# hasnainfarid/Mujoco_Gymnasium_Environments

Hardware: AMD Instinct MI355X
Metric: env steps/sec (whole node), humanoid_soccer 4096 envs/GPU at 1/2/4/8 MI355X (higher is better)
Workload: dtype f64

## Files before the change

mujoco_gymnasium_environments_amd/csrc/mgx_api.hip:

```cpp
#include <hip/hip_runtime.h>

#include <cmath>
#include <cstdio>
#include <cstring>
#include <map>
#include <mutex>
#include <string>
#include <vector>

#include "mgx_task_host.h"

using namespace mgx;

MGX_PROF_SETTER(mgx_prof_set_buffer)

namespace {
thread_local std::string g_err;
}

namespace mgx {
int host_fail(int code, const std::string& msg) {
  g_err = msg;
  return code;
}
// ... 237 lines not shown
    L.hess = u0;
    L.con_pos = endA;
    L.con_frame = align_up(L.con_pos + 3 * max_ncon, al);
    endA = std::max(align_up(L.con_frame + 9 * max_ncon, al), align_up(u0 + (efcg ? nv * (nv + 1) / 2 : nv * nv), al));
  }
  int endB = align_up(u0 + L.chunk_rows * L.Bstride, al);
  L.reals = endA > endB ? endA : endB;
  int q = 0;
  auto takei = [&](int n) { int r = q; q = align_up(q + (n > 0 ? n : 1), 4); return r; };
  L.con_geom = takei(2 * max_ncon);
  L.carry_ints = q;
  L.con_pair = takei(max_ncon);
  L.act_list = takei(max_active);
  L.efc_type = takei(max_nefc); L.efc_id = takei(max_nefc);
  L.con_efcadr = takei(1);
  if (d->solver == 2 && takei(4) != team_off(L)) abort();
  L.ints = q;
  L.bytes = L.reals * real_bytes + L.ints * 4;
  (void)vec_end;
  return L;
}

Layout make_staged_layout(const mgx_model_desc* d, int real_bytes, int max_ncon, int max_nefc, int max_active,
                          int gcon) {
  Layout L{};
  int p = 0;
  const int al = 16 / real_bytes;
  auto a = [&](int n) { return align_up(n > 0 ? n : 1, al); };
  auto take = [&](int n) { int r = p; p += a(n); return r; };
  const int nb = d->nbody, nv = d->nv, nj = d->njnt, ng = d->ngeom;
  L.max_ncon = max_ncon; L.max_nefc = max_nefc; L.max_active = max_active;
  L.staged = 1;
  L.late_geom = 1;
  L.cfs = 3;
  L.qpos = take(d->nq); L.qvel = take(nv); L.ctrl = take(d->nu);
  L.xpos = take(3 * nb); L.xquat = take(4 * nb); L.subtree_com = take(3 * nb);
  L.qLD = take(d->nM); L.con_dist = take(max_ncon);
  L.carry_lds = p;
  L.con_mu = take(max_ncon); L.xfrc = take(6 * nb); L.qMH = take(d->nM);
  L.carry_reals = p;
  p = L.carry_lds;
  const int nvw = nv > 64 ? 128 : 64;
  L.vec0 = take(nvw); L.vec1 = take(nvw); L.vec2 = take(nvw); L.vec3 = take(nvw);
  L.cdof = take(6 * nv);
  L.efc = take(1); L.efc_margin = take(1); L.efc_blk = take(1);
  L.cvel = take(6 * nb);
  const int R = p;
  L.xipos = R; L.cinert = L.xipos + a(3 * nb); L.crb = L.cinert + a(10 * nb);
  const int dead = L.crb + a(10 * nb);
  L.xmat = dead; L.ximat = L.xmat + a(9 * nb); L.xaxis = L.ximat + a(9 * nb); L.xanchor = L.xaxis + a(3 * nj);
  const int endA1 = L.xanchor + a(3 * nj);
  L.cdof_dot = dead; L.cfrc = L.cdof_dot + a(6 * nv); L.act_force = L.cfrc + a(6 * nb);
  L.xfrc_lds = L.act_force + a(d->nu);
  const int endA2 = L.xfrc_lds + a(6 * nb);
  const int ecap = std::min(max_nefc, align_up(2 * nj, 4));
  const int nlist = std::max(max_active, ecap);
  L.geom_xpos = R; L.geom_xmat = L.geom_xpos + a(3 * ng);
  L.con_frame = L.geom_xmat + a(9 * ng);
  L.gcon = gcon;
  L.con_pos = gcon ? 0 : L.con_frame + a(3 * max_ncon);
  L.act_union = L.con_frame + a(3 * max_ncon) + (gcon ? 0 : a(3 * max_ncon));
  const int endC = L.act_union + a((nlist * 4 + real_bytes - 1) / real_bytes);
  L.cacc = a(12 * nb) <= L.con_frame - R ? R : endC;
  const int endD = L.cacc + a(12 * nb);
  L.reals = std::max(std::max(endA1, endA2), std::max(endC, endD));
  L.rowc = 0; L.rk = 0; L.hess = 0;
  L.Bstride = nv | 1; L.Bmat = R; L.chunk_rows = 0; L.gB = 0; L.gB_stride = 0; L.tchunk = 0;
  int q = 0;
  auto takei = [&](int n) { int r = q; q = align_up(q + (n > 0 ? n : 1), 4); return r; };
  L.con_geom = takei(2 * max_ncon);
  L.carry_ints = q;
  L.con_pair = takei(max_ncon);
  L.act_list = 0; L.efc_id = 0;
  L.efc_type = takei(1);
  L.con_efcadr = takei(1);
  L.ints = q;
  L.bytes = L.reals * real_bytes + L.ints * 4;
  return L;
}

Layout finisher_layout(const Layout& S, int real_bytes) {
  Layout L = S;
  const int nvw = S.vec1 - S.vec0;
  L.vec0 = S.carry_reals; L.vec1 = L.vec0 + nvw; L.vec2 = L.vec1 + nvw; L.vec3 = L.vec2 + nvw;
  L.carry_lds = S.carry_reals;
  L.reals = L.vec3 + nvw;
  L.ints = S.carry_ints;
  L.bytes = L.reals * real_bytes + L.ints * 4;
  return L;
}

template <typename T>
struct Builder {
  std::vector<char> host;
  std::vector<std::pair<size_t, const void**>> fix;
  size_t add(const void* src, size_t bytes, const void** slot) {
    size_t off = (host.size() + 15) / 16 * 16;
    host.resize(off + (bytes ? bytes : 16));
    if (bytes) memcpy(host.data() + off, src, bytes);
    fix.push_back({off, slot});
    return off;
  }
  template <typename S>
  void ints(const S* src, size_t n, const int** slot) {
    std::vector<int> v(n ? n : 1, 0);
    for (size_t i = 0; i < n; i++) v[i] = (int)src[i];
    add(v.data(), v.size() * 4, (const void**)slot);
  }
// ... 24 lines not shown
    depth[b] = (int)path.size();
    for (int c = 0; c < depth[b]; c++) chain[b * MGX_MAX_DEPTH + c] = path[depth[b] - 1 - c];
  }
  std::vector<int> chainlen(nv), anc(nv * MGX_MAX_DEPTH, -1), ancadr(nv * MGX_MAX_DEPTH, 0);
  std::vector<uint64_t> ancmask(nv, 0), ancmask_hi(nv, 0);
  for (int k = 0; k < nv; k++) {
    int t = 0;
    for (int j = k; j >= 0; j = d->dof_parentid[j], t++) {
      if (t >= MGX_MAX_DEPTH) return host_fail(MGX_E_CAPACITY, "dof chain longer than MGX_MAX_DEPTH");
      anc[k * MGX_MAX_DEPTH + t] = j;
      ancadr[k * MGX_MAX_DEPTH + t] = d->dof_Madr[j];
      if (j != k) {
        if (j < 64) ancmask[k] |= 1ull << j;
        else ancmask_hi[k] |= 1ull << (j - 64);
      }
    }
    chainlen[k] = t;
  }
  B.ints(d->body_parentid, nb, &M.body_parentid); B.ints(d->body_rootid, nb, &M.body_rootid);
  B.ints(d->body_jntnum, nb, &M.body_jntnum); B.ints(d->body_jntadr, nb, &M.body_jntadr);
  B.ints(d->body_dofnum, nb, &M.body_dofnum); B.ints(d->body_dofadr, nb, &M.body_dofadr);
  B.ints(d->body_subtree_end, nb, &M.body_subtree_end); B.ints(chain.data(), chain.size(), &M.body_chain);
  B.ints(depth.data(), nb, &M.body_depth);
  B.add(d->body_dofmask, sizeof(uint32_t) * nb * d->nmaskword, (const void**)&M.body_dofmask);
  B.reals(d->body_pos, 3 * nb, &M.body_pos); B.reals(d->body_quat, 4 * nb, &M.body_quat);
  B.reals(d->body_ipos, 3 * nb, &M.body_ipos); B.reals(d->body_iquat, 4 * nb, &M.body_iquat);
  B.reals(d->body_mass, nb, &M.body_mass); B.reals(d->body_inertia, 3 * nb, &M.body_inertia);
  B.reals(d->body_invweight0, 2 * nb, &M.body_invweight0);
  B.ints(d->jnt_type, nj, &M.jnt_type); B.ints(d->jnt_bodyid, nj, &M.jnt_bodyid);
  B.ints(d->jnt_qposadr, nj, &M.jnt_qposadr); B.ints(d->jnt_dofadr, nj, &M.jnt_dofadr);
  B.ints(d->jnt_limited, nj, &M.jnt_limited);
  B.reals(d->jnt_pos, 3 * nj, &M.jnt_pos); B.reals(d->jnt_axis, 3 * nj, &M.jnt_axis);
  B.reals(d->jnt_range, 2 * nj, &M.jnt_range); B.reals(d->jnt_stiffness, nj, &M.jnt_stiffness);
  B.reals(d->jnt_margin, nj, &M.jnt_margin); B.reals(d->jnt_solref, 2 * nj, &M.jnt_solref);
  B.reals(d->jnt_solimp, 5 * nj, &M.jnt_solimp);
  B.ints(d->dof_bodyid, nv, &M.dof_bodyid); B.ints(d->dof_jntid, nv, &M.dof_jntid);
  B.ints(d->dof_parentid, nv, &M.dof_parentid); B.ints(d->dof_Madr, nv, &M.dof_Madr);
  B.ints(chainlen.data(), nv, &M.dof_chainlen); B.ints(anc.data(), anc.size(), &M.dof_anc);
  B.add(ancmask.data(), 8 * ancmask.size(), (const void**)&M.dof_ancmask);
  B.add(ancmask_hi.data(), 8 * ancmask_hi.size(), (const void**)&M.dof_ancmask_hi);
  B.ints(ancadr.data(), ancadr.size(), &M.dof_ancadr);
  B.reals(d->dof_armature, nv, &M.dof_armature); B.reals(d->dof_damping, nv, &M.dof_damping);
  B.reals(d->dof_invweight0, nv, &M.dof_invweight0);
  B.ints(d->geom_type, ng, &M.geom_type); B.ints(d->geom_bodyid, ng, &M.geom_bodyid);
  B.reals(d->geom_size, 3 * ng, &M.geom_size); B.reals(d->geom_pos, 3 * ng, &M.geom_pos);
  B.reals(d->geom_quat, 4 * ng, &M.geom_quat); B.reals(d->geom_rbound, ng, &M.geom_rbound);
// ... 241 lines not shown
  };
  h.pgs_lds_rows = get("MGX_PGS_LDS_ROWS", 0);
  h.rk_lds_rows = get("MGX_RK_LDS_ROWS", 0);
  h.pgs_single = get("MGX_PGS_SINGLE", 0);
  h.pgs_lds_b = get("MGX_PGS_LDS_B", MGX_PGS_LDS_B) != 0;
  h.pgs_arena = get("MGX_PGS_ARENA", 0);
  h.pgs_lds_pad = get("MGX_PGS_LDS_PAD", 0);
  h.pgs_wide_lds = get("MGX_PGS_WIDE_LDS", 1);
  h.pgs_spw = get("MGX_PGS_SPW", 0);
  h.pgs_prio_rows = get("MGX_PGS_PRIO_ROWS", 0);
  h.pgs_split_blocks = get("MGX_PGS_SPLIT_BLOCKS", -1);
  h.tight_bp = get("MGX_TIGHT_BROADPHASE", -1);
  h.pgs_wpc = get("MGX_PGS_WPC", 4);
  if (h.pgs_wpc < 4 || h.pgs_wpc > 16) h.pgs_wpc = 4;
  h.side_stream = get("MGX_SIDE_STREAM", 1) != 0;
  h.bank_stream = get("MGX_BANK_STREAM", -1);
  if (h.bank_stream < -1 || h.bank_stream > 2) h.bank_stream = 0;
  h.tail_finish = get("MGX_TAIL_FINISH", -1);
  if (h.tail_finish < -1 || h.tail_finish > 1) h.tail_finish = 0;
  h.tail_factor = get("MGX_TAIL_FACTOR", 1);
  if (h.tail_factor < 0 || h.tail_factor > 2) h.tail_factor = 1;
  h.gcon = get("MGX_GCON", 1);
  h.rows_lds = get("MGX_ROWS_LDS", 0);
  return h;
}

SideStream* mgx::side_stream(hipStream_t st) {
  static std::mutex mu;
  static std::map<std::pair<hipStream_t, int>, SideStream*> cache;
  int dev = 0;
  if (hipGetDevice(&dev) != hipSuccess) return nullptr;
  std::lock_guard<std::mutex> lock(mu);
  auto key = std::make_pair(st, dev);
  auto it = cache.find(key);
  if (it != cache.end()) return it->second;
  SideStream* x = new SideStream{};
  if (hipStreamCreateWithFlags(&x->s, hipStreamNonBlocking) != hipSuccess ||
      hipEventCreateWithFlags(&x->rows, hipEventDisableTiming) != hipSuccess ||
      hipEventCreateWithFlags(&x->big, hipEventDisableTiming) != hipSuccess) {
    delete x;
    x = nullptr;
  }
  cache[key] = x;
  return x;
}

// ... 217 lines not shown
  }
  if (const char* v = getenv("MGX_MAX_NCON")) {
    if (atoi(v) < max_ncon) { delete m; return host_fail(MGX_E_ARG, "MGX_MAX_NCON below the model's contact capacity"); }
    max_ncon = atoi(v);
  }
  if (max_nefc > 1024 || max_ncon > 512) { delete m; return host_fail(MGX_E_CAPACITY, "capacity above 1024 rows / 512 contacts"); }
  max_nefc = (max_nefc + 3) & ~3;
  if (max_nefc < 4 || max_ncon < 1) { delete m; return host_fail(MGX_E_ARG, "row / contact capacity too small"); }
  int rb = precision == MGX_F32 ? 4 : 8;
  int max_active = d->npair <= 256 ? 128 : (d->npair < 768 ? d->npair : 768);
  m->staged_ok = d->integrator == 0 && d->solver == 0 && max_nefc <= 64 * MGX_EFC_SLOTS && condim13 &&
                 d->nv <= 56;
  m->staged_rk_ok = d->integrator == 1 && d->solver == 0 && condim13 && d->nv > 48 && d->nv <= 64 &&
                    max_nefc <= 1024 && max_ncon <= 192;
  const bool mono_lds_rows = !(d->layout_flags & MGX_ROWS_IN_SCRATCH);
  const int mono_nefc = m->staged_ok && mono_lds_rows && max_nefc > 192 ? 192
                        : (m->staged_rk_ok && max_nefc > 512 ? 512 : max_nefc);
  const int mono_ncon = m->staged_ok && mono_lds_rows && max_ncon > 64 ? 64 : max_ncon;
  m->L = make_layout(d, rb, mono_ncon, mono_nefc, max_active);
  if (m->L.bytes > 160 * 1024 || (d->layout_flags & MGX_ROWS_IN_SCRATCH))
    m->L = make_layout(d, rb, mono_ncon, mono_nefc, max_active, true);
  const bool any_staged = m->staged_ok || m->staged_rk_ok;
  m->Ls = make_staged_layout(d, rb, max_ncon, any_staged ? max_nefc : 4, m->staged_ok ? 128 : max_active,
                             m->hooks.gcon);
  m->Lf = finisher_layout(m->Ls, rb);
  {
    const int tight = m->hooks.tight_bp >= 0 ? (m->hooks.tight_bp != 0) : (d->npair > MGX_TIGHT_BROADPHASE_PAIRS);
    m->L.tight_bp = m->Ls.tight_bp = m->Lf.tight_bp = tight;
  }
  int rc;
  if (precision == MGX_F32) {
    rc = build_model<float>(d, device, m, m->mf);
    m->mf.L = m->L; m->mfs = m->mf; m->mfs.L = m->Ls; m->mff = m->mf; m->mff.L = m->Lf;
  } else {
    rc = build_model<double>(d, device, m, m->md);
    m->md.L = m->L; m->mds = m->md; m->mds.L = m->Ls; m->mdf = m->md; m->mdf.L = m->Lf;
  }
  if (rc != MGX_OK) { delete m; return rc; }
  if (m->L.bytes > 160 * 1024) { delete m; return host_fail(MGX_E_CAPACITY, "per-env LDS exceeds 160 KiB"); }
  int r2 = step_kernels_configure(m);
  if (r2 != MGX_OK) { delete m; return r2; }
  r2 = forward_kernels_configure(m);
  if (r2 != MGX_OK) { delete m; return r2; }
  r2 = dyn_kernels_configure(m);
  if (r2 != MGX_OK) { delete m; return r2; }
  r2 = ik_kernels_configure(m);
  if (r2 != MGX_OK) { delete m; return r2; }
// ... 139 lines not shown
```

mujoco_gymnasium_environments_amd/csrc/mgx_common.h:

```cpp
#pragma once
#include <hip/hip_runtime.h>
#include <stdint.h>

#define MGX_WAVE 64
#define MGX_MAX_NV 64
#define MGX_MAX_NV_WIDE 128
#define MGX_MAX_NBODY 64
#define MGX_MAX_DEPTH 16
#define MGX_MAX_CONPAIR 8
#define MGX_TIGHT_BROADPHASE_PAIRS 200
#define MGX_EFC_SLOTS 6

namespace mgx {

enum { JFREE = 0, JBALL = 1, JSLIDE = 2, JHINGE = 3 };
enum { GPLANE = 0, GHFIELD = 1, GSPHERE = 2, GCAPSULE = 3, GELLIPSOID = 4, GCYLINDER = 5, GBOX = 6 };
enum { C_LIMIT_JOINT = 3, C_CONTACT_FRICTIONLESS = 5, C_CONTACT_PYRAMIDAL = 6 };

struct Layout {
  int qpos, qvel, ctrl, xfrc, xpos, xquat, xmat, xipos, ximat, subtree_com, cinert, crb, cvel, cfrc;
  int xaxis, xanchor, cdof, cdof_dot, qLD, qMH, vec0, vec1, vec2, vec3, geom_xpos, geom_xmat, act_force, cacc, rowc;
  int con_dist, con_pos, con_frame, con_mu;
  int efc, efc_margin, efc_blk;
  int Bmat, Bstride;
  int reals;
  int con_geom, con_pair, act_list, efc_type, efc_id, con_efcadr;
  int ints;
  int bytes;
  int max_ncon, max_nefc, max_active;
  int staged, carry_reals, carry_ints, chunk_rows;
  int rk;
  int gB, gB_stride;
  int tchunk;
  int hess;
  int act_union;
  int carry_lds;
  int late_geom, cfs;
  int tight_bp;
  int xfrc_lds;
  int gcon;
};
__host__ __device__ inline int mgx_align(int x, int a) { return (x + a - 1) / a * a; }
__host__ __device__ inline int gb_efc_off(const Layout& L, int real_bytes) {
  return mgx_align(L.max_nefc * L.Bstride, 16 / real_bytes);
}
__host__ __device__ inline int gb_efm_off(const Layout& L, int real_bytes) {
  return gb_efc_off(L, real_bytes) + mgx_align(8 * L.max_nefc, 16 / real_bytes);
}
__host__ __device__ inline int team_off(const Layout& L) { return L.con_efcadr + 4; }

template <typename T>
struct DevModel {
  int nq, nv, nu, nbody, njnt, ngeom, npair, nM, nmaskword;
  int solver, integrator, cone, iterations;
  int has_damping;
  T timestep, tolerance, impratio, meaninertia, gravity[3];
  const int *body_parentid, *body_rootid, *body_jntnum, *body_jntadr, *body_dofnum, *body_dofadr;
  const int *body_subtree_end, *body_chain, *body_depth;
  const uint32_t *body_dofmask;
  const T *body_pos, *body_quat, *body_ipos, *body_iquat, *body_mass, *body_inertia, *body_invweight0;
  const int *jnt_type, *jnt_bodyid, *jnt_qposadr, *jnt_dofadr, *jnt_limited;
  const T *jnt_pos, *jnt_axis, *jnt_range, *jnt_stiffness, *jnt_margin, *jnt_solref, *jnt_solimp;
  const int *dof_bodyid, *dof_jntid, *dof_parentid, *dof_Madr, *dof_chainlen, *dof_anc;
  const uint64_t *dof_ancmask;
  const uint64_t *dof_ancmask_hi;
  const int *dof_ancadr;
  const T *dof_armature, *dof_damping, *dof_invweight0;
  const int *geom_type, *geom_bodyid;
  const T *geom_size, *geom_pos, *geom_quat, *geom_rbound;
  const int *pair_geom, *pair_condim;
  const int* pair_bpi;
  const T* pair_bpr;
  const T* geom_obb;
  const T *pair_friction, *pair_margin, *pair_gap, *pair_solref, *pair_solimp;
  const int *actuator_trnid, *actuator_ctrllimited, *actuator_forcelimited;
  const T *actuator_gear, *actuator_ctrlrange, *actuator_forcerange, *actuator_gainprm, *actuator_biasprm;
  const T *qpos0, *qpos_spring;
  Layout L;
};

#ifdef MGX_PROFILE
static __device__ unsigned long long* g_mgx_prof = nullptr;
#define MGX_PROF_SETTER(name)                                                                     \
  extern "C" int name(void* p) {                                                                 \
    unsigned long long* q = (unsigned long long*)p;                                               \
    return hipMemcpyToSymbol(HIP_SYMBOL(mgx::g_mgx_prof), &q, sizeof(q)) == hipSuccess ? 0 : -3; \
  }
#define MGX_STAMP_DECL unsigned long long _mgx_t0 = __builtin_amdgcn_s_memtime();
#define MGX_STAMP(slot)                                                                 \
  do {                                                                                  \
    __builtin_amdgcn_sched_barrier(0);                                                  \
    unsigned long long _t = __builtin_amdgcn_s_memtime();                               \
    if (g_mgx_prof && threadIdx.x == 0) g_mgx_prof[blockIdx.x * 32 + (slot)] += _t - _mgx_t0; \
    _mgx_t0 = _t;                                                                       \
    __builtin_amdgcn_sched_barrier(0);                                                  \
  } while (0)
#else
#define MGX_PROF_SETTER(name)
#define MGX_STAMP_DECL
#define MGX_STAMP(slot) do {} while (0)
// ... 244 lines not shown
```

mujoco_gymnasium_environments_amd/csrc/mgx_internal.h:

```cpp
#pragma once
#include <hip/hip_runtime.h>

#include <string>
#include <type_traits>

#include "../../include/mgx.h"
#include "mgx_bipedal.h"
#include "mgx_construction.h"
#include "mgx_dancing.h"
#include "mgx_martial.h"
#include "mgx_parkour.h"
#include "mgx_staged.h"
#include "mgx_bank.h"

namespace mgx {
struct Hooks {
  int pgs_lds_rows = 0;
  int rk_lds_rows = 0;
  int pgs_single = 0;
  int pgs_lds_b = 0;
  int pgs_arena = 0;
  int pgs_lds_pad = 0;
  int pgs_wide_lds = 1;
  int pgs_spw = 0;
  int pgs_wpc = 4;
  int pgs_prio_rows = 0;
  int pgs_split_blocks = -1;
  int tight_bp = -1;
  int side_stream = 1;
  int bank_stream = 0;
  int tail_finish = -1;
  int tail_factor = 1;
  int gcon = 1;
  int rows_lds = 0;
};
Hooks read_hooks();
struct RayState;
struct SensorState;
}

struct mgx_model {
  mgx::Hooks hooks;
  int precision;
  int device;
  void* dbuf = nullptr;
  size_t dbytes = 0;
  mgx::DevModel<float> mf, mfs, mff;
  mgx::DevModel<double> md, mds, mdf;
  mgx::Layout L, Ls, Lf;
  bool soccer_ok = false;
  mgx::SoccerIds<float> sf;
  mgx::SoccerIds<double> sd;
  bool parkour_ok = false;
  mgx::ParkourIds<float> pkf;
  mgx::ParkourIds<double> pkd;
  bool martial_ok = false;
  mgx::MartialIds ma;
// ... 145 lines not shown
```

mujoco_gymnasium_environments_amd/csrc/mgx_pgs.hip:

```cpp
#include "mgx_internal.h"

namespace mgx {

int pgs_lanes() {
  static const int lanes = [] {
    const char* v = getenv("MGX_PGS_LPS");
    const int x = v ? atoi(v) : MGX_PGS_LPS;
    return x == 64 ? 64 : 16;
  }();
  return lanes;
}
template <typename T, int LPS, bool BLDS, bool SQG = false>
static void launch_lps(const Pipe& P, int slots, int lds, hipStream_t st, int maxit, T tol, T scale, int big,
                       int spw_hook, int spw_force = 0, int part = 0) {
  const int spw = spw_force ? spw_force : spw_hook ? spw_hook : 64 / LPS;
  int grid = (slots + (spw < 0 ? -spw : spw) - 1) / (spw < 0 ? -spw : spw);
  if (part == 1) grid = slots < MGX_TAIL_HEAVY_GRID ? slots : MGX_TAIL_HEAVY_GRID;
  switch ((P.dpl + LPS / 8 - 1) / (LPS / 8)) {
#define MGX_PGS_CASE(E)                                                                                          \
    case E:                                                                                                     \
      hipLaunchKernelGGL((k_pgs_groups<T, E, LPS, BLDS, SQG>), dim3(grid), dim3(64), lds, st, P, maxit, tol, scale, spw, \
                         big, part);                                                                            \
      break;
    MGX_PGS_CASE(1)
// ... 297 lines not shown
```

mujoco_gymnasium_environments_amd/csrc/mgx_physics.h:

```cpp
#pragma once
#include "mgx_collide.h"

namespace mgx {

template <typename T>
struct Env {
  T *qpos, *qvel, *ctrl, *xfrc, *xpos, *xquat, *xmat, *xipos, *ximat, *subtree_com, *cinert, *crb, *cvel, *cfrc;
  T *xaxis, *xanchor, *cdof, *cdof_dot, *qLD, *qMH, *vec0, *vec1, *vec2, *vec3, *geom_xpos, *geom_xmat, *act_force, *cacc, *rowc;
  T *con_dist, *con_pos, *con_frame, *con_mu;
  T *efc, *efc_margin, *efc_blk;
  T *Bm;
  int Bs;
  T *rk;
  T *hess;
  int *con_geom, *con_pair, *act_list, *efc_type, *efc_id, *con_efcadr;
  int ncon, nefc, niter, overflow;
  int nw;
  int* ctl;
  T qacc_ws, qfrc_applied, qfrc_smooth, qacc_smooth, qacc, qfrc_constraint, diaginv, time;
  int chainlen, madr;
  uint64_t ancmask;
  int qmh_done;
  T qmh_di;
};

template <typename T, bool GB = false, bool EG = false>
__device__ __forceinline__ void env_bind(const DevModel<T>& m, Env<T>& e, char* smem, T* gB = nullptr) {
  T* R = reinterpret_cast<T*>(smem);
  const Layout& L = m.L;
  e.qpos = R + L.qpos; e.qvel = R + L.qvel; e.ctrl = R + L.ctrl; e.xfrc = R + L.xfrc;
  e.xpos = R + L.xpos; e.xquat = R + L.xquat; e.xmat = R + L.xmat; e.xipos = R + L.xipos;
  e.ximat = R + L.ximat; e.subtree_com = R + L.subtree_com; e.cinert = R + L.cinert; e.crb = R + L.crb;
  e.cvel = R + L.cvel; e.cfrc = R + L.cfrc; e.xaxis = R + L.xaxis; e.xanchor = R + L.xanchor;
  e.cdof = R + L.cdof; e.cdof_dot = R + L.cdof_dot; e.qLD = R + L.qLD; e.qMH = R + L.qMH;
  e.vec0 = R + L.vec0; e.vec1 = R + L.vec1; e.vec2 = R + L.vec2; e.vec3 = R + L.vec3; e.geom_xpos = R + L.geom_xpos;
  e.geom_xmat = R + L.geom_xmat; e.act_force = R + L.act_force; e.cacc = R + L.cacc; e.rowc = R + L.rowc; e.con_dist = R + L.con_dist;
  e.con_pos = R + L.con_pos; e.con_frame = R + L.con_frame; e.con_mu = R + L.con_mu; e.efc = R + L.efc;
  e.efc_margin = R + L.efc_margin; e.efc_blk = R + L.efc_blk; e.Bs = L.Bstride;
  if constexpr (EG) { e.efc = gB + gb_efc_off(L, sizeof(T)); e.efc_margin = gB + gb_efm_off(L, sizeof(T)); }
  if constexpr (GB) e.Bm = gB;
  else e.Bm = R + L.Bmat;
  e.rk = R + L.rk;
  e.hess = R + L.hess;
  int* I = reinterpret_cast<int*>(R + L.reals);
  e.con_geom = I + L.con_geom; e.con_pair = I + L.con_pair;
  e.act_list = L.act_union > 0 ? reinterpret_cast<int*>(R + L.act_union) : I + L.act_list;
  e.efc_type = I + L.efc_type; e.con_efcadr = I + L.con_efcadr;
#ifdef MGX_TEAM
  e.nw = blockDim.x >> 6;
  e.ctl = I + team_off(L);
#else
  e.nw = 1;
  e.ctl = nullptr;
#endif
  e.efc_id = L.staged ? e.act_list : I + L.efc_id;
  if (L.carry_lds < L.carry_reals) { e.xfrc = nullptr; e.qMH = nullptr; e.con_mu = nullptr; }
  if (L.gcon) e.con_pos = nullptr;
  int l = lane_id();
  e.chainlen = l < m.nv ? m.dof_chainlen[l] : 0;
  e.madr = l < m.nv ? m.dof_Madr[l] : 0;
  e.ancmask = l < m.nv ? m.dof_ancmask[l] : 0ull;
// ... 30 lines not shown
}

template <typename T>
__device__ __forceinline__ void reset_env(const DevModel<T>& m, Env<T>& e) {
  int l = lane_id();
  wsync();
  for (int k = l; k < m.nq; k += 64) e.qpos[k] = m.qpos0[k];
  for (int k = l; k < m.nv; k += 64) e.qvel[k] = 0;
  for (int k = l; k < m.nu; k += 64) e.ctrl[k] = 0;
  for (int k = l; k < 6 * m.nbody; k += 64) e.xfrc[k] = 0;
  e.qacc_ws = 0;
  e.qfrc_applied = 0;
  e.time = 0;
  wsync();
}

template <typename T>
__device__ __forceinline__ bool any_bad(const T* x, int n) {
  bool b = false;
  for (int k = lane_id(); k < n; k += 64) b |= isbad(x[k]);
  return ballot(b) != 0ull;
}

template <typename T>
__device__ __forceinline__ void body_pose_step(const DevModel<T>& m, Env<T>& e, int i, T* pos, T* quat, T* mat, bool store_joints) {
  int ja = m.body_jntadr[i], jn = m.body_jntnum[i];
  if (jn == 1 && m.jnt_type[ja] == JFREE) {
    int a = m.jnt_qposadr[ja];
    pos[0] = e.qpos[a]; pos[1] = e.qpos[a + 1]; pos[2] = e.qpos[a + 2];
    quat[0] = e.qpos[a + 3]; quat[1] = e.qpos[a + 4]; quat[2] = e.qpos[a + 5]; quat[3] = e.qpos[a + 6];
    normalize4(quat);
    if (store_joints) {
      for (int k = 0; k < 3; k++) { e.xanchor[3 * ja + k] = pos[k]; e.xaxis[3 * ja + k] = m.jnt_axis[3 * ja + k]; }
    }
  } else {
    T np[3], nq[4];
    mulmatvec3(np, mat, m.body_pos + 3 * i);
    for (int k = 0; k < 3; k++) np[k] += pos[k];
    mulquat(nq, quat, m.body_quat + 4 * i);
    for (int j = ja; j < ja + jn; j++) {
      int a = m.jnt_qposadr[j];
      T xaxis[3], xanchor[3];
      rotvecquat(xaxis, m.jnt_axis + 3 * j, nq);
      rotvecquat(xanchor, m.jnt_pos + 3 * j, nq);
      for (int k = 0; k < 3; k++) xanchor[k] += np[k];
      int t = m.jnt_type[j];
      if (t == JSLIDE) {
        T s = e.qpos[a] - m.qpos0[a];
        for (int k = 0; k < 3; k++) np[k] += xaxis[k] * s;
      } else if (t == JHINGE || t == JBALL) {
        T ql[4], v[3];
        if (t == JBALL) { ql[0] = e.qpos[a]; ql[1] = e.qpos[a + 1]; ql[2] = e.qpos[a + 2]; ql[3] = e.qpos[a + 3]; normalize4(ql); }
        else axisangle2quat(ql, m.jnt_axis + 3 * j, e.qpos[a] - m.qpos0[a]);
        mulquat(nq, nq, ql);
        rotvecquat(v, m.jnt_pos + 3 * j, nq);
        for (int k = 0; k < 3; k++) np[k] = xanchor[k] - v[k];
      }
      if (store_joints) for (int k = 0; k < 3; k++) { e.xaxis[3 * j + k] = xaxis[k]; e.xanchor[3 * j + k] = xanchor[k]; }
    }
    pos[0] = np[0]; pos[1] = np[1]; pos[2] = np[2];
    quat[0] = nq[0]; quat[1] = nq[1]; quat[2] = nq[2]; quat[3] = nq[3];
  }
  normalize4(quat);
  quat2mat(mat, quat);
}

template <typename T, bool FROMQ>
__device__ __forceinline__ void geom_poses(const DevModel<T>& m, Env<T>& e);

template <typename T>
__device__ __forceinline__ void kinematics(const DevModel<T>& m, Env<T>& e) {
  int l = lane_id();
  for (int b = l; b < m.nbody; b += 64) {
    T pos[3] = {0, 0, 0}, quat[4] = {1, 0, 0, 0}, mat[9] = {1, 0, 0, 0, 1, 0, 0, 0, 1};
    int depth = m.body_depth[b];
    for (int c = 0; c < depth; c++) {
      int i = m.body_chain[b * MGX_MAX_DEPTH + c];
      body_pose_step(m, e, i, pos, quat, mat, i == b);
    }
    for (int k = 0; k < 3; k++) e.xpos[3 * b + k] = pos[k];
    for (int k = 0; k < 4; k++) e.xquat[4 * b + k] = quat[k];
    for (int k = 0; k < 9; k++) e.xmat[9 * b + k] = mat[k];
    T q[4];
    T ip[3];
    mulmatvec3(ip, mat, m.body_ipos + 3 * b);
    for (int k = 0; k < 3; k++) e.xipos[3 * b + k] = ip[k] + pos[k];
    mulquat(q, quat, m.body_iquat + 4 * b);
    quat2mat(e.ximat + 9 * b, q);
  }
  wsync();
  if (!m.L.late_geom) geom_poses<T, false>(m, e);
}

template <typename T, bool FROMQ>
__device__ __forceinline__ void geom_poses(const DevModel<T>& m, Env<T>& e) {
  const int l = lane_id();
  for (int g = l; g < m.ngeom; g += 64) {
    int b = m.geom_bodyid[g];
    T q[4], gp[3];
    if constexpr (FROMQ) {
      T bm[9];
// ... 636 lines not shown
  }
  T act = 0;
  for (int u = 0; u < m.nu; u++)
    if (m.jnt_dofadr[m.actuator_trnid[u]] == d) act += m.actuator_gear[u] * e.act_force[u];
  T xf = 0;
  for (int i = 1; i < m.nbody; i++) {
    const T* f = e.xfrc + 6 * i;
    if (f[0] == 0 && f[1] == 0 && f[2] == 0 && f[3] == 0 && f[4] == 0 && f[5] == 0) continue;
    if (!body_has_dof(m, i, d)) continue;
    int r = m.body_rootid[i];
    const T* cd = e.cdof + 6 * d;
    T off[3] = {e.xipos[3 * i] - e.subtree_com[3 * r], e.xipos[3 * i + 1] - e.subtree_com[3 * r + 1],
                e.xipos[3 * i + 2] - e.subtree_com[3 * r + 2]}, t[3];
    cross3(t, cd, off);
    xf += (cd[3] + t[0]) * f[0] + (cd[4] + t[1]) * f[1] + (cd[5] + t[2]) * f[2] + cd[0] * f[3] + cd[1] * f[4] + cd[2] * f[5];
  }
  return passive - bias + applied + act + xf;
}
template <typename T>
__device__ __forceinline__ T dof_force(const DevModel<T>& m, const Env<T>& e, int d) {
  return dof_force_applied(m, e, d, e.qfrc_applied);
}

template <typename T>
__device__ __forceinline__ void velocity_bodies(const DevModel<T>& m, Env<T>& e) {
  int l = lane_id();
  for (int b = l; b < m.nbody; b += 64) {
    T cvel[6] = {0, 0, 0, 0, 0, 0};
    int depth = m.body_depth[b];
    for (int c = 0; c < depth; c++) {
      int i = m.body_chain[b * MGX_MAX_DEPTH + c];
      int bda = m.body_dofadr[i], nd = m.body_dofnum[i];
      bool own = i == b;
      for (int j = 0; j < nd; j++) {
        int dof = bda + j;
        int t = m.jnt_type[m.dof_jntid[dof]];
        if (t == JFREE) {
          if (own) for (int q = 0; q < 18; q++) e.cdof_dot[6 * dof + q] = 0;
          for (int q = 0; q < 3; q++)
            for (int k = 0; k < 6; k++) cvel[k] += e.cdof[6 * (dof + q) + k] * e.qvel[dof + q];
          if (own) for (int q = 3; q < 6; q++) crossmotion(e.cdof_dot + 6 * (dof + q), cvel, e.cdof + 6 * (dof + q));
          for (int q = 3; q < 6; q++)
            for (int k = 0; k < 6; k++) cvel[k] += e.cdof[6 * (dof + q) + k] * e.qvel[dof + q];
          j += 5;
        } else if (t == JBALL) {
          if (own) for (int q = 0; q < 3; q++) crossmotion(e.cdof_dot + 6 * (dof + q), cvel, e.cdof + 6 * (dof + q));
          for (int q = 0; q < 3; q++)
            for (int k = 0; k < 6; k++) cvel[k] += e.cdof[6 * (dof + q) + k] * e.qvel[dof + q];
          j += 2;
        } else {
          if (own) crossmotion(e.cdof_dot + 6 * dof, cvel, e.cdof + 6 * dof);
          for (int k = 0; k < 6; k++) cvel[k] += e.cdof[6 * dof + k] * e.qvel[dof];
        }
      }
    }
    for (int k = 0; k < 6; k++) e.cvel[6 * b + k] = cvel[k];
  }
  for (int u = l; u < m.nu; u += 64) {
    int j = m.actuator_trnid[u];
    T ctrl = e.ctrl[u];
    if (m.actuator_ctrllimited[u]) ctrl = clampv(ctrl, m.actuator_ctrlrange[2 * u], m.actuator_ctrlrange[2 * u + 1]);
    T g = m.actuator_gear[u];
    T len = g * e.qpos[m.jnt_qposadr[j]], vel = g * e.qvel[m.jnt_dofadr[j]];
    const T* gp = m.actuator_gainprm + 3 * u;
    const T* bp = m.actuator_biasprm + 3 * u;
    T f = gp[0] * ctrl + bp[0] + bp[1] * len + bp[2] * vel;
    if (m.actuator_forcelimited[u]) f = clampv(f, m.actuator_forcerange[2 * u], m.actuator_forcerange[2 * u + 1]);
    e.act_force[u] = f;
  }
  wsync();
  for (int b = l; b < m.nbody; b += 64) {
    if (b == 0) { for (int k = 0; k < 6; k++) e.cfrc[k] = 0; continue; }
    T cacc[6] = {0, 0, 0, -m.gravity[0], -m.gravity[1], -m.gravity[2]};
    int depth = m.body_depth[b];
    for (int c = 0; c < depth; c++) {
      int i = m.body_chain[b * MGX_MAX_DEPTH + c];
      int bda = m.body_dofadr[i], nd = m.body_dofnum[i];
      for (int j = 0; j < nd; j++)
        for (int k = 0; k < 6; k++) cacc[k] += e.cdof_dot[6 * (bda + j) + k] * e.qvel[bda + j];
    }
    T f[6], tmp[6], tmp1[6];
    mulinertvec(f, e.cinert + 10 * b, cacc);
    mulinertvec(tmp, e.cinert + 10 * b, e.cvel + 6 * b);
    crossforce(tmp1, e.cvel + 6 * b, tmp);
    for (int k = 0; k < 6; k++) e.cfrc[6 * b + k] = f[k] + tmp1[k];
  }
  wsync();
  for (int b = l; b < m.nbody; b += 64) {
    T acc[6] = {0, 0, 0, 0, 0, 0};
    if (b > 0) {
      int end = m.body_subtree_end[b];
      for (int i = b; i < end; i++)
        for (int k = 0; k < 6; k++) acc[k] += e.cfrc[6 * i + k];
    }
    for (int k = 0; k < 6; k++) e.crb[10 * b + k] = acc[k];
  }
  wsync();
}

template <typename T>
// ... 760 lines not shown
```

mujoco_gymnasium_environments_amd/csrc/mgx_pk_staged.hip:

```cpp
#include "mgx_internal.h"

using namespace mgx;

namespace mgx {

constexpr int PK_LPS = 16;
constexpr int PK_OBS = 95;
constexpr int PK_SPLIT_BLOCKS = 56;
enum { PK_SUBSTEPS = 10 };

template <typename T>
struct ParkourBank {
  typedef ParkourIds<T> Ids;
  typedef mgx_parkour_env EnvT;
  struct Draws { T d0, d1; };
  static constexpr int OBS = PK_OBS, DRAWS = 2;
  static constexpr bool STG = false, STEP_COUNTS = false;
  static constexpr int FIX_CTR = 5;
  __device__ static int fix_entry(int env) { return env; }
  __device__ static int fix_env(int entry) { return entry; }
  __device__ __forceinline__ static Draws draws(Env<T>& e, const Ids&, const T* host, uint64_t seed, uint32_t genv,
                                                uint32_t episode) {
    if (host) return Draws{host[0], host[1]};
    parkour_philox_draws(seed, genv, episode, e.vec1);
// ... 295 lines not shown
```

mujoco_gymnasium_environments_amd/csrc/mgx_rk_staged.hip:

```cpp
#include "mgx_internal.h"

using namespace mgx;

MGX_PROF_SETTER(mgx_prof_set_buffer_rk_staged)

namespace mgx {

constexpr int RK_NCS = 3;
constexpr int RK_LPS = 16;
constexpr int RK_EPL = 4;
constexpr int RK_OBS = 102;
enum { RK_IDLE = 0, RK_ACTIVE = 1 };

template <typename T>
struct RkCarry {
  T *q0, *x, *v, *f, *t;
};
template <typename T>
__device__ __forceinline__ RkCarry<T> rk_carry(const DevModel<T>& m, const Pipe& P, int slot) {
  T* b = P.at<T>(P.o_rk) + (size_t)slot * P.rk_stride;
  const int nq4 = (m.nq + 3) & ~3;
  RkCarry<T> r;
  r.q0 = b;
  r.x = b + nq4;
// ... 520 lines not shown
```

mujoco_gymnasium_environments_amd/csrc/mgx_staged.h:

```cpp
#pragma once
#include "mgx_soccer.h"

namespace mgx {

#define MGX_SCAL 5
#define MGX_SQ(k, i) (4 * (k) + (i))
#define MGX_TW 4
__host__ __device__ constexpr int mgx_twl(bool dofb) { return dofb ? 4 : 8; }
#define MGX_PGS_LPS 16
#define MGX_PGS_LDS_B 0
#define MGX_PGS_RING 2
#define MGX_PGS_RING_LDS 2
#define MGX_PGS_LDS_ROWS 192
#define MGX_PGS_SPLIT_BLOCKS 40
#define MGX_BANK_STREAM 1
#define MGX_TAIL_FINISH 1
#define MGX_TAIL_HEAVY_GRID 1024
#define MGX_TAIL_DEFER_GRID 256
#define MGX_PGS_WIDE_GRID 256
#define MGX_PGS_WIDE_LDS_GRID 32
#define MGX_PGS_ARENA_F64 49152
#define MGX_PGS_ARENA_F32 32768
enum { FIX_RESET = 2 };

// ... 357 lines not shown
  e.qacc_smooth = solve_M(m, e, e.qLD, e.diaginv, e.qfrc_smooth);
  MGX_STAMP(4);
  if (m.L.late_geom) geom_poses<T, true>(m, e);
  collision(m, e);
  MGX_STAMP(5);
  int nlim, ncf;
  const int ne = rows_plan(m, e, &nlim, &ncf);
  e.nefc = ne;
  MGX_STAMP(6);
  const bool dl = l < nv;
  int boff = 32;
  if (ne > 0) {
    const T dinvs = dl ? sqrt(e.diaginv) : (T)0;
    T* scal = P.at<T>(P.o_scal) + (size_t)slot * P.maxE * MGX_SCAL;
    T* Bo = P.at<T>(P.o_B) + (size_t)slot * P.bcap;
    uint32_t* blk = P.at<uint32_t>(P.o_blk) + (size_t)slot * (P.maxE / 4) * MGX_TW;
    const int nlim4 = (nlim + 3) & ~3;
    if (dl) { e.vec1[l] = e.qacc_smooth; e.vec2[l] = e.qacc_ws; }
    wsync();
    if (ncf > 0) {
      for (int b = l; b < m.nbody; b += 64) {
        T a[12] = {0, 0, 0, 0, 0, 0, 0, 0, 0, 0, 0, 0};
        int depth = m.body_depth[b];
        for (int c = 0; c < depth; c++) {
          int i = m.body_chain[b * MGX_MAX_DEPTH + c];
          int bda = m.body_dofadr[i], nd = m.body_dofnum[i];
          for (int jd = bda; jd < bda + nd; jd++) {
            T xs = e.vec1[jd], xw = e.vec2[jd];
            const T* cd = e.cdof + 6 * jd;
            for (int q = 0; q < 6; q++) { a[q] += cd[q] * xs; a[6 + q] += cd[q] * xw; }
          }
        }
        for (int q = 0; q < 12; q++) e.cacc[12 * b + q] = a[q];
      }
      wsync();
    }
    rows_impedance(m, e, ne, nlim, nlim4, scal);
    ContactMeta<T> cm, cm2, cm3;
    contact_meta(m, e, ncf, cm);
    if constexpr (NCS > 1) contact_meta(m, e, ncf, cm2, 64);
    if constexpr (NCS > 2) contact_meta(m, e, ncf, cm3, 128);
    __threadfence();
    wsync();
    for (int r0 = 0; r0 < ne; r0 += 4)
      build_block<T, NCS, DOFB>(m, e, P, r0, nlim, nlim4, cm, cm2, cm3, dinvs, scal, blk, Bo, boff);
  }
  MGX_STAMP(7);
  T* cr = P.at<T>(P.o_carry) + (size_t)slot * P.carry_stride;
  for (int k = l; k < m.L.carry_lds; k += 64) cr[k] = reinterpret_cast<T*>(e.qpos)[k - m.L.qpos];
// ... 663 lines not shown
```

Baseline: 1.905 million.

## Pack per-chain kinematic records and precompute joint quaternions in a prepass

Builds packed per-chain-entry records (body/joint indices, body pos/quat, dof ranges with joint kind) and per-joint records on the host so kinematics, velocity and bias passes read them as vector loads instead of chasing several indirect arrays. Adds a joint prepass that computes each joint's local quaternion or slide offset once into a scratch region, instead of recomputing it for every body whose chain passes through that joint. It is enabled by default in the staged, PGS and parkour kernels, and adds an extra sync plus scratch LDS aliased onto the cinert area, which is only used if it fits.

```diff
diff --git a/mujoco_gymnasium_environments_amd/csrc/mgx_api.hip b/mujoco_gymnasium_environments_amd/csrc/mgx_api.hip
--- a/mujoco_gymnasium_environments_amd/csrc/mgx_api.hip
+++ b/mujoco_gymnasium_environments_amd/csrc/mgx_api.hip
@@ -283,7 +283,7 @@
 }
 
 Layout make_staged_layout(const mgx_model_desc* d, int real_bytes, int max_ncon, int max_nefc, int max_active,
-                          int gcon) {
+                          int gcon, int chain_rec) {
   Layout L{};
   int p = 0;
   const int al = 16 / real_bytes;
@@ -309,6 +309,8 @@
   const int R = p;
   L.xipos = R; L.cinert = L.xipos + a(3 * nb); L.crb = L.cinert + a(10 * nb);
   const int dead = L.crb + a(10 * nb);
+  L.jq = L.cinert;
+  L.chain_rec = 4 * nj <= dead - L.cinert ? chain_rec : chain_rec & ~1;
   L.xmat = dead; L.ximat = L.xmat + a(9 * nb); L.xaxis = L.ximat + a(9 * nb); L.xanchor = L.xaxis + a(3 * nj);
   const int endA1 = L.xanchor + a(3 * nj);
   L.cdof_dot = dead; L.cfrc = L.cdof_dot + a(6 * nv); L.act_force = L.cfrc + a(6 * nb);
@@ -345,6 +347,7 @@
   const int nvw = S.vec1 - S.vec0;
   L.vec0 = S.carry_reals; L.vec1 = L.vec0 + nvw; L.vec2 = L.vec1 + nvw; L.vec3 = L.vec2 + nvw;
   L.carry_lds = S.carry_reals;
+  L.chain_rec = 0;
   L.reals = L.vec3 + nvw;
   L.ints = S.carry_ints;
   L.bytes = L.reals * real_bytes + L.ints * 4;
@@ -415,6 +418,37 @@
   B.ints(d->body_dofnum, nb, &M.body_dofnum); B.ints(d->body_dofadr, nb, &M.body_dofadr);
   B.ints(d->body_subtree_end, nb, &M.body_subtree_end); B.ints(chain.data(), chain.size(), &M.body_chain);
   B.ints(depth.data(), nb, &M.body_depth);
+  {
+    std::vector<int> hi(4 * (size_t)nb * MGX_MAX_DEPTH, 0), dofw((size_t)nb * MGX_MAX_DEPTH, 0), ji(4 * (size_t)nj, 0);
+    std::vector<double> hr(8 * (size_t)nb * MGX_MAX_DEPTH, 0.0), jr(8 * (size_t)nj, 0.0);
+    for (int b = 0; b < nb; b++)
+      for (int c = 0; c < depth[b]; c++) {
+        const size_t e = (size_t)b * MGX_MAX_DEPTH + c;
+        const int i = chain[e], ja = d->body_jntadr[i], jn = d->body_jntnum[i];
+        hi[4 * e] = i; hi[4 * e + 1] = jn; hi[4 * e + 2] = ja;
+        hi[4 * e + 3] = jn == 1 && d->jnt_type[ja] == JFREE ? d->jnt_qposadr[ja] : -1;
+        for (int k = 0; k < 3; k++) hr[8 * e + k] = d->body_pos[3 * i + k];
+        for (int k = 0; k < 4; k++) hr[8 * e + 3 + k] = d->body_quat[4 * i + k];
+        const int da = d->body_dofadr[i], dn = d->body_dofnum[i];
+        int kind = -1;
+        for (int q = da; q < da + dn; q++) {
+          const int t = d->jnt_type[d->dof_jntid[q]];
+          const int kt = t == JFREE || t == JBALL ? t : JHINGE;
+          kind = kind < 0 || kind == kt ? kt : 4;
+        }
+        if (dn > 255 || (dn > 0 && da > 255)) return host_fail(MGX_E_CAPACITY, "body dof range beyond the chain records");
+        dofw[e] = dn > 0 ? (da | dn << 8 | (kind < 0 ? JHINGE : kind) << 16) : 0;
+      }
+    for (int j = 0; j < nj; j++) {
+      const int a = d->jnt_qposadr[j];
+      ji[4 * j] = d->jnt_type[j]; ji[4 * j + 1] = a;
+      for (int k = 0; k < 3; k++) { jr[8 * j + k] = d->jnt_axis[3 * j + k]; jr[8 * j + 3 + k] = d->jnt_pos[3 * j + k]; }
+      jr[8 * j + 6] = d->qpos0[a];
+    }
+    B.ints(hi.data(), hi.size(), &M.kin_hi); B.ints(ji.data(), ji.size(), &M.kin_ji);
+    B.ints(dofw.data(), dofw.size(), &M.chain_dofw);
+    B.reals(hr.data(), hr.size(), &M.kin_hr); B.reals(jr.data(), jr.size(), &M.kin_jr);
+  }
   B.add(d->body_dofmask, sizeof(uint32_t) * nb * d->nmaskword, (const void**)&M.body_dofmask);
   B.reals(d->body_pos, 3 * nb, &M.body_pos); B.reals(d->body_quat, 4 * nb, &M.body_quat);
   B.reals(d->body_ipos, 3 * nb, &M.body_ipos); B.reals(d->body_iquat, 4 * nb, &M.body_iquat);
@@ -702,6 +736,7 @@
   if (h.tail_factor < 0 || h.tail_factor > 2) h.tail_factor = 1;
   h.gcon = get("MGX_GCON", 1);
   h.rows_lds = get("MGX_ROWS_LDS", 0);
+  h.chain_records = get("MGX_CHAIN_RECORDS", 3) & 3;
   return h;
 }
 
@@ -965,7 +1000,7 @@
     m->L = make_layout(d, rb, mono_ncon, mono_nefc, max_active, true);
   const bool any_staged = m->staged_ok || m->staged_rk_ok;
   m->Ls = make_staged_layout(d, rb, max_ncon, any_staged ? max_nefc : 4, m->staged_ok ? 128 : max_active,
-                             m->hooks.gcon);
+                             m->hooks.gcon, m->hooks.chain_records);
   m->Lf = finisher_layout(m->Ls, rb);
   {
     const int tight = m->hooks.tight_bp >= 0 ? (m->hooks.tight_bp != 0) : (d->npair > MGX_TIGHT_BROADPHASE_PAIRS);
diff --git a/mujoco_gymnasium_environments_amd/csrc/mgx_common.h b/mujoco_gymnasium_environments_amd/csrc/mgx_common.h
--- a/mujoco_gymnasium_environments_amd/csrc/mgx_common.h
+++ b/mujoco_gymnasium_environments_amd/csrc/mgx_common.h
@@ -39,6 +39,7 @@
   int tight_bp;
   int xfrc_lds;
   int gcon;
+  int chain_rec, jq;
 };
 __host__ __device__ inline int mgx_align(int x, int a) { return (x + a - 1) / a * a; }
 __host__ __device__ inline int gb_efc_off(const Layout& L, int real_bytes) {
@@ -76,6 +77,8 @@
   const int *actuator_trnid, *actuator_ctrllimited, *actuator_forcelimited;
   const T *actuator_gear, *actuator_ctrlrange, *actuator_forcerange, *actuator_gainprm, *actuator_biasprm;
   const T *qpos0, *qpos_spring;
+  const int *kin_hi, *kin_ji, *chain_dofw;
+  const T *kin_hr, *kin_jr;
   Layout L;
 };
 
diff --git a/mujoco_gymnasium_environments_amd/csrc/mgx_internal.h b/mujoco_gymnasium_environments_amd/csrc/mgx_internal.h
--- a/mujoco_gymnasium_environments_amd/csrc/mgx_internal.h
+++ b/mujoco_gymnasium_environments_amd/csrc/mgx_internal.h
@@ -33,6 +33,7 @@
   int tail_factor = 1;
   int gcon = 1;
   int rows_lds = 0;
+  int chain_records = 3;
 };
 Hooks read_hooks();
 struct RayState;
diff --git a/mujoco_gymnasium_environments_amd/csrc/mgx_pgs.hip b/mujoco_gymnasium_environments_amd/csrc/mgx_pgs.hip
--- a/mujoco_gymnasium_environments_amd/csrc/mgx_pgs.hip
+++ b/mujoco_gymnasium_environments_amd/csrc/mgx_pgs.hip
@@ -1,3 +1,4 @@
+#define MGX_CHAIN_RECORDS 1
 #include "mgx_internal.h"
 
 namespace mgx {
diff --git a/mujoco_gymnasium_environments_amd/csrc/mgx_physics.h b/mujoco_gymnasium_environments_amd/csrc/mgx_physics.h
--- a/mujoco_gymnasium_environments_amd/csrc/mgx_physics.h
+++ b/mujoco_gymnasium_environments_amd/csrc/mgx_physics.h
@@ -9,6 +9,7 @@
   T *xaxis, *xanchor, *cdof, *cdof_dot, *qLD, *qMH, *vec0, *vec1, *vec2, *vec3, *geom_xpos, *geom_xmat, *act_force, *cacc, *rowc;
   T *con_dist, *con_pos, *con_frame, *con_mu;
   T *efc, *efc_margin, *efc_blk;
+  T *jq;
   T *Bm;
   int Bs;
   T *rk;
@@ -37,6 +38,7 @@
   e.geom_xmat = R + L.geom_xmat; e.act_force = R + L.act_force; e.cacc = R + L.cacc; e.rowc = R + L.rowc; e.con_dist = R + L.con_dist;
   e.con_pos = R + L.con_pos; e.con_frame = R + L.con_frame; e.con_mu = R + L.con_mu; e.efc = R + L.efc;
   e.efc_margin = R + L.efc_margin; e.efc_blk = R + L.efc_blk; e.Bs = L.Bstride;
+  e.jq = R + L.jq;
   if constexpr (EG) { e.efc = gB + gb_efc_off(L, sizeof(T)); e.efc_margin = gB + gb_efm_off(L, sizeof(T)); }
   if constexpr (GB) e.Bm = gB;
   else e.Bm = R + L.Bmat;
@@ -113,8 +115,55 @@
   return ballot(b) != 0ull;
 }
 
-template <typename T>
-__device__ __forceinline__ void body_pose_step(const DevModel<T>& m, Env<T>& e, int i, T* pos, T* quat, T* mat, bool store_joints) {
+__device__ __forceinline__ int chain_rec(const Layout& L) {
+#ifdef MGX_CHAIN_RECORDS
+  return L.chain_rec;
+#else
+  (void)L;
+  return 0;
+#endif
+}
+__device__ __forceinline__ void load_rec8(float* r, const float* p) {
+  const float4 a = reinterpret_cast<const float4*>(p)[0], b = reinterpret_cast<const float4*>(p)[1];
+  r[0] = a.x; r[1] = a.y; r[2] = a.z; r[3] = a.w; r[4] = b.x; r[5] = b.y; r[6] = b.z; r[7] = b.w;
+}
+__device__ __forceinline__ void load_rec8(double* r, const double* p) {
+  const double2* q = reinterpret_cast<const double2*>(p);
+  const double2 a = q[0], b = q[1], c = q[2], d = q[3];
+  r[0] = a.x; r[1] = a.y; r[2] = b.x; r[3] = b.y; r[4] = c.x; r[5] = c.y; r[6] = d.x; r[7] = d.y;
+}
+
+template <typename T>
+__device__ __forceinline__ void joint_prepass(const DevModel<T>& m, Env<T>& e, bool rec) {
+  for (int j = lane_id(); j < m.njnt; j += 64) {
+    int t, a;
+    T ax[3], q0;
+    if (rec) {
+      const int2 tj = *reinterpret_cast<const int2*>(m.kin_ji + 4 * j);
+      T r[8];
+      load_rec8(r, m.kin_jr + 8 * j);
+      t = tj.x; a = tj.y; ax[0] = r[0]; ax[1] = r[1]; ax[2] = r[2]; q0 = r[6];
+    } else {
+      t = m.jnt_type[j]; a = m.jnt_qposadr[j];
+      ax[0] = m.jnt_axis[3 * j]; ax[1] = m.jnt_axis[3 * j + 1]; ax[2] = m.jnt_axis[3 * j + 2];
+      q0 = t == JFREE ? (T)0 : m.qpos0[a];
+    }
+    T* o = e.jq + 4 * j;
+    if (t == JSLIDE) {
+      o[0] = e.qpos[a] - q0;
+    } else if (t == JHINGE || t == JBALL) {
+      T ql[4];
+      if (t == JBALL) { ql[0] = e.qpos[a]; ql[1] = e.qpos[a + 1]; ql[2] = e.qpos[a + 2]; ql[3] = e.qpos[a + 3]; normalize4(ql); }
+      else axisangle2quat(ql, ax, e.qpos[a] - q0);
+      o[0] = ql[0]; o[1] = ql[1]; o[2] = ql[2]; o[3] = ql[3];
+    }
+  }
+  wsync();
+}
+
+template <typename T>
+__device__ __forceinline__ void body_pose_step(const DevModel<T>& m, Env<T>& e, int i, T* pos, T* quat, T* mat, bool store_joints,
+                                               bool pre = false) {
   int ja = m.body_jntadr[i], jn = m.body_jntnum[i];
   if (jn == 1 && m.jnt_type[ja] == JFREE) {
     int a = m.jnt_qposadr[ja];
@@ -137,11 +186,12 @@
       for (int k = 0; k < 3; k++) xanchor[k] += np[k];
       int t = m.jnt_type[j];
       if (t == JSLIDE) {
-        T s = e.qpos[a] - m.qpos0[a];
+        T s = pre ? e.jq[4 * j] : e.qpos[a] - m.qpos0[a];
         for (int k = 0; k < 3; k++) np[k] += xaxis[k] * s;
       } else if (t == JHINGE || t == JBALL) {
         T ql[4], v[3];
-        if (t == JBALL) { ql[0] = e.qpos[a]; ql[1] = e.qpos[a + 1]; ql[2] = e.qpos[a + 2]; ql[3] = e.qpos[a + 3]; normalize4(ql); }
+        if (pre) { ql[0] = e.jq[4 * j]; ql[1] = e.jq[4 * j + 1]; ql[2] = e.jq[4 * j + 2]; ql[3] = e.jq[4 * j + 3]; }
+        else if (t == JBALL) { ql[0] = e.qpos[a]; ql[1] = e.qpos[a + 1]; ql[2] = e.qpos[a + 2]; ql[3] = e.qpos[a + 3]; normalize4(ql); }
         else axisangle2quat(ql, m.jnt_axis + 3 * j, e.qpos[a] - m.qpos0[a]);
         mulquat(nq, nq, ql);
         rotvecquat(v, m.jnt_pos + 3 * j, nq);
@@ -156,18 +206,79 @@
   quat2mat(mat, quat);
 }
 
+template <typename T>
+__device__ __forceinline__ void body_pose_step_rec(const DevModel<T>& m, Env<T>& e, const int4 h, const T* hr, T* pos, T* quat,
+                                                   T* mat, bool store_joints, bool pre) {
+  int ja = h.z, jn = h.y;
+  if (h.w >= 0) {
+    int a = h.w;
+    pos[0] = e.qpos[a]; pos[1] = e.qpos[a + 1]; pos[2] = e.qpos[a + 2];
+    quat[0] = e.qpos[a + 3]; quat[1] = e.qpos[a + 4]; quat[2] = e.qpos[a + 5]; quat[3] = e.qpos[a + 6];
+    normalize4(quat);
+    if (store_joints) {
+      for (int k = 0; k < 3; k++) { e.xanchor[3 * ja + k] = pos[k]; e.xaxis[3 * ja + k] = m.kin_jr[8 * ja + k]; }
+    }
+  } else {
+    T np[3], nq[4];
+    mulmatvec3(np, mat, hr);
+    for (int k = 0; k < 3; k++) np[k] += pos[k];
+    mulquat(nq, quat, hr + 3);
+    for (int j = ja; j < ja + jn; j++) {
+      const int2 tj = *reinterpret_cast<const int2*>(m.kin_ji + 4 * j);
+      const T* jr = m.kin_jr + 8 * j;
+      int a = tj.y;
+      T xaxis[3], xanchor[3];
+      rotvecquat(xaxis, jr, nq);
+      rotvecquat(xanchor, jr + 3, nq);
+      for (int k = 0; k < 3; k++) xanchor[k] += np[k];
+      int t = tj.x;
+      if (t == JSLIDE) {
+        T s = pre ? e.jq[4 * j] : e.qpos[a] - jr[6];
+        for (int k = 0; k < 3; k++) np[k] += xaxis[k] * s;
+      } else if (t == JHINGE || t == JBALL) {
+        T ql[4], v[3];
+        if (pre) { ql[0] = e.jq[4 * j]; ql[1] = e.jq[4 * j + 1]; ql[2] = e.jq[4 * j + 2]; ql[3] = e.jq[4 * j + 3]; }
+        else if (t == JBALL) { ql[0] = e.qpos[a]; ql[1] = e.qpos[a + 1]; ql[2] = e.qpos[a + 2]; ql[3] = e.qpos[a + 3]; normalize4(ql); }
+        else axisangle2quat(ql, jr, e.qpos[a] - jr[6]);
+        mulquat(nq, nq, ql);
+        rotvecquat(v, jr + 3, nq);
+        for (int k = 0; k < 3; k++) np[k] = xanchor[k] - v[k];
+      }
+      if (store_joints) for (int k = 0; k < 3; k++) { e.xaxis[3 * j + k] = xaxis[k]; e.xanchor[3 * j + k] = xanchor[k]; }
+    }
+    pos[0] = np[0]; pos[1] = np[1]; pos[2] = np[2];
+    quat[0] = nq[0]; quat[1] = nq[1]; quat[2] = nq[2]; quat[3] = nq[3];
+  }
+  normalize4(quat);
+  quat2mat(mat, quat);
+}
+
 template <typename T, bool FROMQ>
 __device__ __forceinline__ void geom_poses(const DevModel<T>& m, Env<T>& e);
 
 template <typename T>
 __device__ __forceinline__ void kinematics(const DevModel<T>& m, Env<T>& e) {
   int l = lane_id();
+  const int cr = chain_rec(m.L);
+  const bool pre = cr & 1;
+  if (pre) joint_prepass(m, e, (cr & 2) != 0);
   for (int b = l; b < m.nbody; b += 64) {
     T pos[3] = {0, 0, 0}, quat[4] = {1, 0, 0, 0}, mat[9] = {1, 0, 0, 0, 1, 0, 0, 0, 1};
     int depth = m.body_depth[b];
-    for (int c = 0; c < depth; c++) {
-      int i = m.body_chain[b * MGX_MAX_DEPTH + c];
-      body_pose_step(m, e, i, pos, quat, mat, i == b);
+    if (cr & 2) {
+      const int4* hi = reinterpret_cast<const int4*>(m.kin_hi) + b * MGX_MAX_DEPTH;
+      const T* hrp = m.kin_hr + 8 * b * MGX_MAX_DEPTH;
+      int4 h = hi[0];
+      for (int c = 0; c < depth; c++) {
+        const int4 hn = hi[c + 1 < depth ? c + 1 : c];
+        body_pose_step_rec(m, e, h, hrp + 8 * c, pos, quat, mat, h.x == b, pre);
+        h = hn;
+      }
+    } else {
+      for (int c = 0; c < depth; c++) {
+        int i = m.body_chain[b * MGX_MAX_DEPTH + c];
+        body_pose_step(m, e, i, pos, quat, mat, i == b, pre);
+      }
     }
     for (int k = 0; k < 3; k++) e.xpos[3 * b + k] = pos[k];
     for (int k = 0; k < 4; k++) e.xquat[4 * b + k] = quat[k];
@@ -850,19 +961,41 @@
   return dof_force_applied(m, e, d, e.qfrc_applied);
 }
 
+struct ChainDofs {
+  int base, cur;
+  bool rec;
+  template <typename T>
+  __device__ __forceinline__ ChainDofs(const DevModel<T>& m, int b, bool rec_) : base(b * MGX_MAX_DEPTH), cur(0), rec(rec_) {
+    if (rec) cur = m.chain_dofw[base];
+  }
+  template <typename T>
+  __device__ __forceinline__ void next(const DevModel<T>& m, int c, int depth, int& bda, int& nd, int& kt) {
+    if (rec) {
+      const int w = cur;
+      if (c + 1 < depth) cur = m.chain_dofw[base + c + 1];
+      bda = w & 255; nd = (w >> 8) & 255; kt = w >> 16;
+    } else {
+      const int i = m.body_chain[base + c];
+      bda = m.body_dofadr[i]; nd = m.body_dofnum[i]; kt = 4;
+    }
+  }
+};
+
 template <typename T>
 __device__ __forceinline__ void velocity_bodies(const DevModel<T>& m, Env<T>& e) {
   int l = lane_id();
+  const bool rec = (chain_rec(m.L) & 2) != 0;
   for (int b = l; b < m.nbody; b += 64) {
     T cvel[6] = {0, 0, 0, 0, 0, 0};
     int depth = m.body_depth[b];
+    ChainDofs cw(m, b, rec);
     for (int c = 0; c < depth; c++) {
-      int i = m.body_chain[b * MGX_MAX_DEPTH + c];
-      int bda = m.body_dofadr[i], nd = m.body_dofnum[i];
-      bool own = i == b;
+      int bda, nd, kt;
+      cw.next(m, c, depth, bda, nd, kt);
+      bool own = c == depth - 1;
       for (int j = 0; j < nd; j++) {
         int dof = bda + j;
-        int t = m.jnt_type[m.dof_jntid[dof]];
+        int t = kt == 4 ? m.jnt_type[m.dof_jntid[dof]] : kt;
         if (t == JFREE) {
           if (own) for (int q = 0; q < 18; q++) e.cdof_dot[6 * dof + q] = 0;
           for (int q = 0; q < 3; q++)
@@ -901,9 +1034,10 @@
     if (b == 0) { for (int k = 0; k < 6; k++) e.cfrc[k] = 0; continue; }
     T cacc[6] = {0, 0, 0, -m.gravity[0], -m.gravity[1], -m.gravity[2]};
     int depth = m.body_depth[b];
+    ChainDofs cw(m, b, rec);
     for (int c = 0; c < depth; c++) {
-      int i = m.body_chain[b * MGX_MAX_DEPTH + c];
-      int bda = m.body_dofadr[i], nd = m.body_dofnum[i];
+      int bda, nd, kt;
+      cw.next(m, c, depth, bda, nd, kt);
       for (int j = 0; j < nd; j++)
         for (int k = 0; k < 6; k++) cacc[k] += e.cdof_dot[6 * (bda + j) + k] * e.qvel[bda + j];
     }
diff --git a/mujoco_gymnasium_environments_amd/csrc/mgx_pk_staged.hip b/mujoco_gymnasium_environments_amd/csrc/mgx_pk_staged.hip
--- a/mujoco_gymnasium_environments_amd/csrc/mgx_pk_staged.hip
+++ b/mujoco_gymnasium_environments_amd/csrc/mgx_pk_staged.hip
@@ -1,3 +1,4 @@
+#define MGX_CHAIN_RECORDS 1
 #include "mgx_internal.h"
 
 using namespace mgx;
diff --git a/mujoco_gymnasium_environments_amd/csrc/mgx_rk_staged.hip b/mujoco_gymnasium_environments_amd/csrc/mgx_rk_staged.hip
--- a/mujoco_gymnasium_environments_amd/csrc/mgx_rk_staged.hip
+++ b/mujoco_gymnasium_environments_amd/csrc/mgx_rk_staged.hip
@@ -1,3 +1,4 @@
+#define MGX_CHAIN_RECORDS 1
 #include "mgx_internal.h"
 
 using namespace mgx;
diff --git a/mujoco_gymnasium_environments_amd/csrc/mgx_staged.h b/mujoco_gymnasium_environments_amd/csrc/mgx_staged.h
--- a/mujoco_gymnasium_environments_amd/csrc/mgx_staged.h
+++ b/mujoco_gymnasium_environments_amd/csrc/mgx_staged.h
@@ -403,9 +403,10 @@
       for (int b = l; b < m.nbody; b += 64) {
         T a[12] = {0, 0, 0, 0, 0, 0, 0, 0, 0, 0, 0, 0};
         int depth = m.body_depth[b];
+        ChainDofs cw(m, b, (chain_rec(m.L) & 2) != 0);
         for (int c = 0; c < depth; c++) {
-          int i = m.body_chain[b * MGX_MAX_DEPTH + c];
-          int bda = m.body_dofadr[i], nd = m.body_dofnum[i];
+          int bda, nd, kt;
+          cw.next(m, c, depth, bda, nd, kt);
           for (int jd = bda; jd < bda + nd; jd++) {
             T xs = e.vec1[jd], xw = e.vec2[jd];
             const T* cd = e.cdof + 6 * jd;
```

Measured after the change: 1.941 million (median of 6 runs). 1.9% higher.
